# jjhbw/GoMILP

Measured on AMD Instinct MI355X. Metric: simplex pivots/sec on 2048x4096 fp64 dense LP, higher is better.
Workload: dtype f64

## Files before the change

### gomilp_amd/csrc/btg_kernels.hip

```cpp
#include <hip/hip_runtime.h>
#include <hip/hip_ext.h>
#include <stdint.h>

#include <algorithm>
#include <type_traits>

#include "device_types.h"
#include "kernels_common.h"
#include "bt_loop.h"

namespace gomilp {

namespace {

struct XWin { double m; unsigned int i; double p0, p1, p2, p3; };
struct BtWinG { double m; unsigned int i; };

}

template <int G, int NT, int RI, int KR, bool STAMP, bool LOOP = false>
__device__ __forceinline__ void bt_innerG_body(const BTArgs &a, const int g, const int nupd = 0) {
    constexpr int NW = NT / 64;
    static_assert(!LOOP || KR == 16 || KR == 24 || KR == 32, "loop mode: KR / 2 lagging + KR / 2 current terms");
    constexpr int KB = LOOP ? KR / 2 : KR;
    static_assert(G == 2 || G == 4 || G == 8 || G == 16, "G");
#ifdef GOMILP_DEBUG
    if (a.fault && g == 1) return;
#endif
    __shared__ double redM[16];
    __shared__ unsigned int redI[16];
    __shared__ double pay[16][4];
    __shared__ int s_ok;
    __shared__ unsigned long long s_acc[STAMP ? 16 : 1][16];
    unsigned long long tprev = 0;
    auto stamp = [&](int seg) {
        if constexpr (STAMP) {
            unsigned long long t;
            __builtin_amdgcn_sched_barrier(0);
            asm volatile("s_memtime %0\n\ts_waitcnt lgkmcnt(0)" : "=s"(t)::"memory");
            __builtin_amdgcn_sched_barrier(0);
            if (seg >= 0 && (threadIdx.x & 63) == 0) s_acc[threadIdx.x >> 6][seg] += t - tprev;
            tprev = t;
        }
    };
    DevState *st = a.st;
    const int tid = threadIdx.x, lane = tid & 63, wv = tid >> 6;
    const int wbase = __builtin_amdgcn_readfirstlane(tid & ~63);
    const int done = __hip_atomic_load(&st->done, __ATOMIC_RELAXED, __HIP_MEMORY_SCOPE_AGENT);
    long long xs = (long long)a.xbuf[0];
    xpair *recs = reinterpret_cast<xpair *>(a.xbuf + kXHeader);
    const double inf = __builtin_inf();
    const unsigned int ldt = (unsigned int)a.ldt;
    const char *Tb = reinterpret_cast<const char *>(a.T);
    auto ldT = [&](unsigned int elem) -> double {
        if constexpr (LOOP) return ld_agent(reinterpret_cast<const double *>(Tb + (elem << 3)));
        else return *reinterpret_cast<const double *>(Tb + (elem << 3));
    };
    auto ld_term = [&](const double *p) -> double { return ld_agent(p); };
    auto st_term = [&](double *p, double v) { st_agent(p, v); };
    auto gidx = [&](int s) -> int { return (s * G + g) * NT + tid; };
    unsigned int myxcc;
    asm volatile("s_getreg_b32 %0, hwreg(HW_REG_XCC_ID)" : "=s"(myxcc));
    myxcc &= 0xFu;
    bool fast = false, first = true;
    double xbv[RI], rv[RI];
    int basv[RI], nbasv[RI];
#pragma unroll
    for (int s = 0; s < RI; s++) {
        const int i = gidx(s);
        xbv[s] = i < a.m ? a.xb[i] : 0.0;
        basv[s] = i < a.m ? a.basic[i] : 0;
        rv[s] = i < a.nn ? a.r[i] : inf;
        nbasv[s] = i < a.nn ? a.nonbasic[i] : 0;
    }
    int cur0 = 0, lag0 = KB, nl = 0;
    const int sel0 = LOOP ? (a.par ? st->tsel2[1] : st->tsel2[0]) : 0;
    const double *hdr_in = a.xbuf + 1 + 5 * (LOOP ? a.par : 0);
    double *hdr_out = a.xbuf + 1 + 5 * (LOOP ? (a.par ^ 1) : 0);
    const unsigned int blk_base = LOOP ? (unsigned int)(unsigned long long)hdr_in[0] : 0u;
    unsigned int upd_base[4];
#pragma unroll
    for (int j = 0; j < 4; j++) upd_base[j] = LOOP ? (unsigned int)(unsigned long long)hdr_in[1 + j] : 0u;
    unsigned int *blk_cnt = reinterpret_cast<unsigned int *>(a.xbuf + kXSync), *upd_cnt = reinterpret_cast<unsigned int *>(a.xbuf + kXSync + 16);
    auto hand_on = [&](int nb) {
        hdr_out[0] = (double)(unsigned int)(blk_base + (unsigned int)G * (unsigned int)nb);
#pragma unroll
        for (int j = 0; j < 4; j++) hdr_out[1 + j] = (double)(unsigned int)(upd_base[j] + (unsigned int)nupd * (unsigned int)(nb > j ? (nb - 1 - j) / 4 + 1 : 0));
    };
    if (done) {
        if constexpr (LOOP) {
            if (tid == 0) {
                if (g == 0) {
                    __hip_atomic_store(&st->kdone2[0], 0, __ATOMIC_RELAXED, __HIP_MEMORY_SCOPE_AGENT);
                    asm volatile("s_waitcnt vmcnt(0)" ::: "memory");
                }
                __hip_atomic_fetch_add(blk_cnt, 1u, __ATOMIC_RELAXED, __HIP_MEMORY_SCOPE_AGENT);
                if (g == 0) {
                    st->tsel2[a.par ^ 1] = sel0;
                    st->loop_blocks = 0;
                    hand_on(1);
                }
            }
        } else if (g == 0 && tid == 0) st->kdone = 0;
        return;
    }
    double ureg[RI][KR], vreg[RI][KR];
#pragma unroll
    for (int s = 0; s < RI; s++) {
#pragma unroll
        for (int j = 0; j < KR; j++) { ureg[s][j] = 0; vreg[s][j] = 0; }
    }
    if constexpr (STAMP) { if (tid < 256) s_acc[tid >> 4][tid & 15] = 0; }
    __syncthreads();
    int kd = 0, status = ST_RUNNING, blands = 0;
    bool dead = false;
    long long trace_len = 0, npiv = 0;
    if (g == 0 && tid == 0) { trace_len = st->trace_len; npiv = st->pivots; }

    auto wave_first_min = [&](const double (&val)[RI]) -> BtWinG {
        double x = val[0];
#pragma unroll
        for (int s = 1; s < RI; s++) x = vmin_f64(x, val[s]);
        BtWinG w;
        w.m = wave_min_f64(x);
        w.i = 0xFFFFFFFFu;
#pragma unroll
        for (int s = RI - 1; s >= 0; s--) {
            const unsigned long long mask = __ballot(val[s] == w.m);
            if (mask) w.i = (unsigned int)((s * G + g) * NT + wbase + __builtin_ctzll(mask));
        }
        return w;
    };
    auto xchg = [&](int which) -> XWin {
        stamp(which * 5 + 0);
        if constexpr (!LOOP) asm volatile("s_waitcnt vmcnt(0)" ::: "memory");
        __syncthreads();
        stamp(which * 5 + 1);
        xs += 1;
        const double seqd = (double)xs;
        const int par = (int)(xs & 1);
        if (wv == 0) {
            double fm, v0;
            unsigned int fi;
            if constexpr (LOOP && (NW == 4 || NW == 8)) {
                const double mw = lane < NW ? redM[lane & (NW - 1)] : inf;
                const double iw = lane < NW ? (double)redI[lane & (NW - 1)] : 4294967295.0;
                double xm = mw;
                xm = vmin_f64(xm, dpp_f64<0xB1>(xm));
                xm = vmin_f64(xm, dpp_f64<0x4E>(xm));
                if constexpr (NW == 8) xm = vmin_f64(xm, dpp_f64<0x141>(xm));
                const bool mine = lane < NW && mw == xm;
                double km = mine ? iw : 4294967295.0;
                km = vmin_f64(km, dpp_f64<0xB1>(km));
                km = vmin_f64(km, dpp_f64<0x4E>(km));
                if constexpr (NW == 8) km = vmin_f64(km, dpp_f64<0x141>(km));
                const unsigned int mk = (unsigned int)(__ballot(mine && iw == km) & ((1ull << NW) - 1ull));
                const int ww = mk ? __builtin_ctz(mk) : 0;
                fm = readlane_f64(mw, ww);
                fi = (unsigned int)readlane_f64(iw, ww);
                v0 = pay[ww][lane < 5 && lane >= 2 ? lane - 2 : 3];
            } else {
                fm = redM[0];
                fi = redI[0];
                v0 = pay[0][lane < 5 && lane >= 2 ? lane - 2 : 3];
#pragma unroll
                for (int w2 = 1; w2 < NW; w2++) {
                    const double mw = redM[w2];
                    const unsigned int iw = redI[w2];
                    const double pw = pay[w2][lane < 5 && lane >= 2 ? lane - 2 : 3];
                    const bool take = (mw < fm) || (mw == fm && iw < fi) || (fm != fm && mw == mw);
                    fm = take ? mw : fm;
                    fi = take ? iw : fi;
                    v0 = take ? pw : v0;
                }
            }
            if (lane < kXSlots) {
                xpair v;
                v.x = seqd;
                v.y = lane == 0 ? fm : lane == 1 ? (double)fi : lane == 5 ? (double)myxcc : v0;
                xstore(recs + ((size_t)(par * G + g) * kXSlots + lane), v, fast);
            }
            if constexpr (STAMP && !LOOP) asm volatile("s_waitcnt vmcnt(0)" ::: "memory");
        }
        stamp(which * 5 + 2);
        for (int dl = 0; dl < a.poll_delay; dl++) __builtin_amdgcn_s_sleep(1);
        if constexpr (G == 16) {
            const int rec = lane & 15, grp = lane >> 4;
            const bool actB = grp < 3;
            const xpair *base = recs + (size_t)par * G * kXSlots + rec * kXSlots;
            const xpair *srcA = base + (grp == 0 ? 0 : grp + 1), *srcB = base + (grp == 0 ? 1 : grp == 1 ? 5 : grp == 2 ? 6 : 0);
            xpair got[2];
            int spins = 0;
            for (;;) {
                XLoad<2>::run(srcA, srcB, got, fast);
                if (__all(got[0].x == seqd && (!actB || got[1].x == seqd))) break;
                if (++spins > kXSpinLimit) { dead = true; break; }
            }
            stamp(which * 5 + 3);
            const double val = got[0].y, val2 = got[1].y;
            double xm = (lane < 16) ? val : inf;
            xm = vmin_f64(xm, dpp_f64<0xB1>(xm));
            xm = vmin_f64(xm, dpp_f64<0x4E>(xm));
            xm = vmin_f64(xm, dpp_f64<0x141>(xm));
            xm = vmin_f64(xm, dpp_f64<0x140>(xm));
            const bool mine = lane < 16 && val == xm;
            const unsigned int mk0 = (unsigned int)(__ballot(mine) & 0xFFFFull);
            int gw;
            double bi;
            if (__builtin_popcount(mk0) == 1) {
                gw = __builtin_ctz(mk0);
                bi = readlane_f64(val2, gw);
            } else {
                double km = mine ? val2 : 4294967295.0;
                km = vmin_f64(km, dpp_f64<0xB1>(km));
                km = vmin_f64(km, dpp_f64<0x4E>(km));
                km = vmin_f64(km, dpp_f64<0x141>(km));
                km = vmin_f64(km, dpp_f64<0x140>(km));
                const unsigned int mk = (unsigned int)(__ballot(mine && val2 == km) & 0xFFFFull);
                gw = mk ? __builtin_ctz(mk) : 0;
                bi = readlane_f64(km, 0);
            }
            XWin r;
            r.m = readlane_f64(xm, 0);
            r.i = (unsigned int)bi;
            r.p0 = readlane_f64(val, 16 + gw);
            r.p1 = readlane_f64(val, 32 + gw);
            r.p2 = readlane_f64(val, 48 + gw);
            r.p3 = readlane_f64(val2, 32 + gw);
            if (first) {
                fast = !dead && __all(grp != 1 || val2 == (double)myxcc);
                first = false;
            }
            stamp(which * 5 + 4);
            return r;
        }
        const bool act = (lane & 7) < G && (lane >> 3) < 7;
        const xpair *src = recs + (size_t)par * G * kXSlots + (act ? (lane & 7) * kXSlots + (lane >> 3) : 0);
        xpair got[1];
        int spins = 0;
        for (;;) {
            XLoad<1>::run(src, got, fast);
            if (__all(!act || got[0].x == seqd)) break;
            if (++spins > kXSpinLimit) { dead = true; break; }
        }
        stamp(which * 5 + 3);
        const double val = got[0].y;
        double xm = (lane < G) ? val : inf;
        xm = vmin_f64(xm, dpp_f64<0xB1>(xm));
        xm = vmin_f64(xm, dpp_f64<0x4E>(xm));
        xm = vmin_f64(xm, dpp_f64<0x141>(xm));
        const double idxl = dpp_f64<0x108>(val);
        const bool mine = lane < G && val == xm;
        double km = mine ? idxl : 4294967295.0;
        km = vmin_f64(km, dpp_f64<0xB1>(km));
        km = vmin_f64(km, dpp_f64<0x4E>(km));
        km = vmin_f64(km, dpp_f64<0x141>(km));
        const unsigned int mk = (unsigned int)(__ballot(mine && idxl == km) & 0xFFull);
        const int gw = mk ? __builtin_ctz(mk) : 0;
        const double bm = readlane_f64(xm, 0), bi = readlane_f64(km, 0);
        XWin r;
        r.m = bm;
        r.i = (unsigned int)bi;
        r.p0 = readlane_f64(val, 16 + gw);
        r.p1 = readlane_f64(val, 24 + gw);
        r.p2 = readlane_f64(val, 32 + gw);
        r.p3 = readlane_f64(val, 48 + gw);
        if (first) {
            fast = !dead && __all(!(act && (lane >> 3) == 5) || val == (double)myxcc);
            first = false;
        }
        stamp(which * 5 + 4);
        return r;
    };
    auto reduce_cols = [&](const double (&val)[RI]) -> XWin {
        const BtWinG w = wave_first_min(val);
#pragma unroll
        for (int s = 0; s < RI; s++)
            if ((unsigned int)gidx(s) == w.i) {
                pay[wv][0] = rv[s];
                pay[wv][1] = (double)nbasv[s];
                pay[wv][3] = vreg[s][0];
            }
        if (lane == 0) { redM[wv] = w.m; redI[wv] = w.i; }
        return xchg(0);
    };
    auto reduce_rows = [&](const double (&val)[RI], const double (&dcol)[RI]) -> XWin {
        const BtWinG w = wave_first_min(val);
#pragma unroll
        for (int s = 0; s < RI; s++)
            if ((unsigned int)gidx(s) == w.i) {
                pay[wv][0] = dcol[s];
                pay[wv][1] = xbv[s];
                pay[wv][2] = (double)basv[s];
                pay[wv][3] = ureg[s][0];
            }
        if (lane == 0) { redM[wv] = w.m; redI[wv] = w.i; }
        return xchg(1);
    };
    auto column = [&](int q, int k, double (&dcol)[RI], double newest) {
        double d0[RI];
#pragma unroll
        for (int s = 0; s < RI; s++) {
            const int i = gidx(s);
            const unsigned int ic = (unsigned int)(i < a.m ? i : a.m - 1);
            d0[s] = ldT(tile_off_g(ic, (unsigned int)q, ldt));
        }
        double vq[KR];
        if constexpr (LOOP) {
            const int l = lane & 31;
            const int trow = l < k ? cur0 + k - 1 - l : lag0 + nl - 1 - (l - k);
            double tv = l < k + nl ? ld_term(a.V + (size_t)trow * a.ldt + q) : 0.0;
            if (l == 0 && k + nl > 0) tv = newest;
            if constexpr (STAMP) { asm volatile("s_waitcnt vmcnt(0)" ::: "memory"); stamp(11); }
#pragma unroll
            for (int jj = 0; jj < KR; jj++) vq[jj] = readlane_f64(tv, jj);
        } else {
#pragma unroll
            for (int jj = 0; jj < KR; jj++) vq[jj] = jj < k ? ld_term(a.V + (size_t)(k - 1 - jj) * a.ldt + q) : 0.0;
        }
#pragma unroll
        for (int s = 0; s < RI; s++) {
            double d;
            if constexpr (LOOP) {
                double acc[4] = {0, 0, 0, 0};
#pragma unroll
                for (int j = 0; j < KR; j++) acc[j & 3] = __builtin_fma(ureg[s][j], vq[j], acc[j & 3]);
                d = d0[s] + ((acc[0] + acc[1]) + (acc[2] + acc[3]));
            } else {
                d = d0[s];
#pragma unroll
                for (int j = 0; j < KR; j++) d = __builtin_fma(ureg[s][j], vq[j], d);
            }
            dcol[s] = gidx(s) < a.m ? d : 0.0;
        }
    };
    auto ratios = [&](const double (&dcol)[RI], double (&mvv)[RI]) {
#pragma unroll
        for (int s = 0; s < RI; s++) {
            const int i = gidx(s);
            double d = -dcol[s];
            if (fabs(d) < 1e-13) d = 0;
            const double quot = div_pos(xbv[s], fabs(d));
            mvv[s] = (d >= 0 || i >= a.m) ? inf : quot;
        }
    };

    int nbe = 0;
    for (int blk = 0; blk < (LOOP ? a.nblocks : 1); blk++) {
    if constexpr (LOOP) {
        if (blk >= 2) {
            if (wv == 0) {
                const int cj = (blk - 2) & 3;
                const unsigned int ub = cj == 0 ? upd_base[0] : cj == 1 ? upd_base[1] : cj == 2 ? upd_base[2] : upd_base[3];
                const bool ok = spin_counter(upd_cnt + 16 * cj * 2, ub + (unsigned int)nupd * (unsigned int)((blk - 2) / 4 + 1), 0);
                if (lane == 0) s_ok = ok ? 1 : 0;
            }
            __syncthreads();
            if (!s_ok) { dead = true; break; }
        }
        Tb = reinterpret_cast<const char *>(((sel0 ^ (blk > 0 ? blk - 1 : 0)) & 1) ? a.Tbuf[1] : a.Tbuf[0]);
        cur0 = (blk & 1) * KB; lag0 = cur0 ^ KB; nl = blk > 0 ? KB : 0;
        if (blk > 0) {
#pragma unroll
            for (int s = 0; s < RI; s++) {
#pragma unroll
                for (int j = KB; j < KR; j++) { ureg[s][j] = 0; vreg[s][j] = 0; }
            }
        }
        kd = 0;
    }
    for (int k = 0; k < a.kmax; k++) {
        stamp(-1);
        const bool forced = (k == 0 && blk == 0 && a.forced_q >= 0);
        int q, p, ent = 0, lea = 0;
        double rq = 0, dpv = 1.0, xbp = 0, unew = 0;
        bool bland = false;
        double dcol[RI];
        if (!forced) {
            const XWin fq = reduce_cols(rv);
            if (dead) break;
            q = (int)fq.i; rq = fq.p0; ent = (int)fq.p1;
            if (fq.i >= (unsigned int)a.nn) { q = 0; rq = __builtin_nan(""); }
            if (a.guard == inf && !(k == 0 && blk == 0 && a.exact_once)) { status = ST_NEED_EXACT; break; }
            if (rq >= -a.tol) { status = ST_OPTIMAL; break; }
            column(q, k, dcol, fq.p3);
            XWin w;
            {
                double mvv[RI];
                ratios(dcol, mvv);
                w = reduce_rows(mvv, dcol);
            }
            if (dead) break;
            p = (int)w.i; dpv = w.p0; xbp = w.p1; lea = (int)w.p2; unew = w.p3;
            const double mv = w.m;
            if (mv == inf || w.i >= (unsigned int)a.m) { status = ST_UNBOUNDED; break; }
            if (a.guard > 0 && (mv <= a.guard || fabs(dpv) <= a.guard) && !(k == 0 && blk == 0 && a.exact_once)) { status = ST_NEED_EXACT; break; }
            if (a.cguard > 0 && fabs(dpv) <= a.cguard && !(k == 0 && blk == 0 && a.exact_once)) { status = ST_NEED_EXACT; break; }
            if (mv <= 0) {
                bland = true;
                blands++;
                int cand = -1;
                bool found = false;
                for (;;) {
                    double fl[RI];
#pragma unroll
                    for (int s = 0; s < RI; s++) {
                        const int j = gidx(s);
                        double rr = rv[s];
                        if (fabs(rr) < 1e-13) rr = 0;
                        fl[s] = (j < a.nn && j > cand && !(rr > -1e-14)) ? 0.0 : inf;
                    }
                    const XWin fc = reduce_cols(fl);
                    if (dead) break;
                    if (fc.m != 0.0) break;
                    cand = (int)fc.i;
                    const double rqc = fc.p0;
                    const int entc = (int)fc.p1;
                    column(cand, k, dcol, fc.p3);
                    XWin w2;
                    {
                        double mvv[RI];
                        ratios(dcol, mvv);
                        w2 = reduce_rows(mvv, dcol);
                    }
                    if (dead) break;
                    if (w2.m == inf || w2.i >= (unsigned int)a.m) { status = ST_UNBOUNDED; break; }
                    if (fabs(w2.m) > 1e-12) {
                        q = cand; p = (int)w2.i; rq = rqc; ent = entc; dpv = w2.p0; xbp = w2.p1; lea = (int)w2.p2; unew = w2.p3;
                        found = true;
                        break;
                    }
                    double gl2[RI];
                    ratios(dcol, gl2);
#pragma unroll
                    for (int s = 0; s < RI; s++) gl2[s] = (gidx(s) < a.m && !(gl2[s] > 1e-12)) ? 0.0 : inf;
                    const XWin gw = reduce_rows(gl2, dcol);
                    if (dead) break;
                    if (gw.m == 0.0) {
                        q = cand; p = (int)gw.i; rq = rqc; ent = entc; dpv = gw.p0; xbp = gw.p1; lea = (int)gw.p2; unew = gw.p3;
                        found = true;
                        break;
                    }
                }
                if (dead || status == ST_UNBOUNDED) break;
                if (!found) { status = ST_BLAND_FAILED; break; }
            }
        } else {
            q = a.forced_q; p = a.forced_p; rq = 0;
            double fl[RI];
#pragma unroll
            for (int s = 0; s < RI; s++) fl[s] = (gidx(s) == q) ? 0.0 : inf;
            const XWin fc = reduce_cols(fl);
            if (dead) break;
            ent = (int)fc.p1;
            if (!a.forced_nocommit) rq = fc.p0;
            column(q, k, dcol, fc.p3);
            double gl2[RI];
#pragma unroll
            for (int s = 0; s < RI; s++) gl2[s] = (gidx(s) == p) ? 0.0 : inf;
            const XWin gw = reduce_rows(gl2, dcol);
            if (dead) break;
            dpv = gw.p0; xbp = gw.p1; lea = (int)gw.p2; unew = gw.p3;
        }
        const double rinv = 1.0 / dpv, nrinv = -rinv;
        const double mult = rq * rinv;
        const double theta = xbp * rinv;
        double *Vk = a.V + (size_t)(cur0 + k) * a.ldt;
        double *Uk = a.U + (size_t)(cur0 + k) * a.ldu;
        const bool commit_lists = !(forced && a.forced_nocommit) || (forced && a.forced_nocommit >= 2);
        double vrow[RI];
#pragma unroll
        for (int s = 0; s < RI; s++) {
            const int j = gidx(s);
            vrow[s] = j < a.ldt ? ldT(tile_off_g((unsigned int)p, (unsigned int)j, ldt)) : 0.0;
        }
        double up[KR];
        if constexpr (LOOP) {
            const int l = lane & 31;
            const int trow = l < k ? cur0 + k - 1 - l : lag0 + nl - 1 - (l - k);
            double tv = l < k + nl ? ld_term(a.U + (size_t)trow * a.ldu + p) : 0.0;
            if (l == 0 && k + nl > 0) tv = unew;
            if constexpr (STAMP) { asm volatile("s_waitcnt vmcnt(0)" ::: "memory"); stamp(12); }
#pragma unroll
            for (int jj = 0; jj < KR; jj++) up[jj] = readlane_f64(tv, jj);
        } else {
#pragma unroll
            for (int jj = 0; jj < KR; jj++) up[jj] = jj < k ? ld_term(a.U + (size_t)(k - 1 - jj) * a.ldu + p) : 0.0;
        }
        if constexpr (LOOP) asm volatile("s_waitcnt vmcnt(0)" ::: "memory");
#pragma unroll
        for (int s = 0; s < RI; s++) {
            const int i = gidx(s);
            if (i < a.ldu) {
                const double u = (i == p) ? rinv - 1.0 : dcol[s] * nrinv;
                if (i < a.m) xbv[s] = (i == p) ? theta : __builtin_fma(-theta, dcol[s], xbv[s]);
                st_term(Uk + i, u);
#pragma unroll
                for (int jj = KR - 1; jj > 0; jj--) ureg[s][jj] = ureg[s][jj - 1];
                ureg[s][0] = u;
                if (i == p && commit_lists) basv[s] = ent;
            }
        }
#pragma unroll
        for (int s = 0; s < RI; s++) {
            const int j = gidx(s);
            if (j < a.ldt) {
                double v;
                if constexpr (LOOP) {
                    double acc[4] = {0, 0, 0, 0};
#pragma unroll
                    for (int jj = 0; jj < KR; jj++) acc[jj & 3] = __builtin_fma(up[jj], vreg[s][jj], acc[jj & 3]);
                    v = vrow[s] + ((acc[0] + acc[1]) + (acc[2] + acc[3]));
                } else {
                    v = vrow[s];
#pragma unroll
                    for (int jj = 0; jj < KR; jj++) v = __builtin_fma(up[jj], vreg[s][jj], v);
                }
                rv[s] = (j == q) ? -mult : __builtin_fma(-mult, v, rv[s]);
                const double vprime = (j == q) ? dpv + 1.0 : v;
                st_term(Vk + j, vprime);
#pragma unroll
                for (int jj = KR - 1; jj > 0; jj--) vreg[s][jj] = vreg[s][jj - 1];
                vreg[s][0] = vprime;
                if (j == q && commit_lists) nbasv[s] = lea;
            }
        }
        if constexpr (STAMP && !LOOP) asm volatile("s_waitcnt vmcnt(0)" ::: "memory");
        stamp(10);
        if (forced && a.forced_nocommit == 3) status = ST_FORCED_DONE;
        if (g == 0 && tid == 0 && !(forced && a.forced_nocommit)) {
            if (a.trace && trace_len < a.trace_cap) {
                DevPivot &tr = a.trace[trace_len];
                tr.phase = a.phase; tr.bland = bland ? 1 : 0; tr.min_idx = q; tr.replace = p; tr.entering = ent; tr.leaving = lea;
            }
            trace_len += 1;
            npiv += 1;
        }
        kd = k + 1;
    }
    nbe = blk + 1;
    if constexpr (LOOP) {
        if (dead) status = ST_XCHG_TIMEOUT;
        asm volatile("s_waitcnt vmcnt(0)" ::: "memory");
        __syncthreads();
        if (tid == 0) {
            if (g == 0) {
                __hip_atomic_store(&st->kdone2[blk & 1], kd, __ATOMIC_RELAXED, __HIP_MEMORY_SCOPE_AGENT);
                if (status != ST_RUNNING) {
                    __hip_atomic_store(&st->status, status, __ATOMIC_RELAXED, __HIP_MEMORY_SCOPE_AGENT);
                    __hip_atomic_store(&st->done, 1, __ATOMIC_RELAXED, __HIP_MEMORY_SCOPE_AGENT);
                }
                asm volatile("s_waitcnt vmcnt(0)" ::: "memory");
            }
            __hip_atomic_fetch_add(blk_cnt, 1u, __ATOMIC_RELAXED, __HIP_MEMORY_SCOPE_AGENT);
        }
        if (status != ST_RUNNING) break;
    }
    }
    if (dead) status = ST_XCHG_TIMEOUT;
    if constexpr (STAMP) {
        if (a.stamps && g == 0 && lane == 0) {
            for (int sg = 0; sg < 16; sg++) a.stamps[wv * 16 + sg] += s_acc[wv][sg];
            if (wv == 0) a.stamps[16 * 16] += (unsigned long long)kd;
        }
    }
#pragma unroll
    for (int s = 0; s < RI; s++) {
        const int i = gidx(s);
        if (i < a.ldt) a.r[i] = i < a.nn ? rv[s] : 0.0;
        if (i < a.ldu) a.xb[i] = xbv[s];
        if (i < a.m) a.basic[i] = basv[s];
        if (i < a.nn) a.nonbasic[i] = nbasv[s];
    }
    if (tid == 0 && (g == 0 || dead)) {
        if (g == 0) {
            st->trace_len = trace_len;
            st->pivots = npiv;
            if constexpr (LOOP) {
                const int napplied = kd > 0 ? nbe : nbe - 1;
                st->tsel2[a.par ^ 1] = sel0 ^ (napplied & 1);
                st->loop_blocks = nbe;
                hand_on(nbe);
            } else {
                st->kdone = kd;
            }
            st->bland_steps += blands;
            a.xbuf[0] = (double)xs;
        }
        if (status != ST_RUNNING) { st->done = 1; st->status = status; }
    }
}

template <int G, int NT, int RI, int KR, bool STAMP = false>
__global__ __launch_bounds__(NT) void k_bt_innerG(BTArgs a) {
    if (blockIdx.x & 7u) return;
    bt_innerG_body<G, NT, RI, KR, STAMP>(a, (int)(blockIdx.x >> 3));
}
template <int G, int NT, int RI, bool STAMP = false, int KB = 8>
__global__ __launch_bounds__(NT) void k_bt_loop(BTArgs a) {
    const int b = (int)blockIdx.x, x = a.xcd & 7;
    const int nupd = (a.upd_cap > 0 && a.upd_cap < (int)gridDim.x - G) ? a.upd_cap : (int)gridDim.x - G;
    if ((b & 7) == x && (b >> 3) < G) { bt_innerG_body<G, NT, RI, 2 * KB, STAMP, true>(a, b >> 3, nupd); return; }
    const int before = b <= x ? 0 : min(G, ((b - x - 1) >> 3) + 1);
    if (b - before >= nupd) return;
    bt_loop_update_role<NT, KB>(a, b - before, nupd, G);
}

template <int G, int NT, int RI, int KR>
__global__ __launch_bounds__(NT) void k_bt_innerG_batch(const BatchLP *__restrict__ lps, const int *__restrict__ ids, const int *__restrict__ count, int xcd_off) {
    const unsigned int x8 = ((blockIdx.x & 7u) + 8u - (unsigned int)xcd_off) & 7u, j = blockIdx.x >> 3;
    const int lpos = (int)((j / G) * 8u + x8);
    if (lpos >= *count) return;
    const BatchLP &lp = lps[ids[lpos]];
    const int stage = lp.stage;
    if (stage == BS_DONE || stage == BS_HOST) return;
    const BTArgs a = lp.bt;
    bt_innerG_body<G, NT, RI, KR, false>(a, (int)(j % G));
}


size_t bt_xbuf_doubles() { return (size_t)kXSync + kXSyncDoubles; }

BtGroupCfg bt_group_cfg(int m, int ldt, int knob) {
    BtGroupCfg c = {0, 0, 0};
    if (knob < 0) return c;
    const int need = m > ldt ? m : ldt;
    auto fits = [&](int G, int nt, int ri) { return (long)G * nt * ri >= need; };
    if (knob == 16) {
        if (need <= 2048) c = {8, 256, 1};
        else if (need <= 4096) c = {8, 512, 1};
        return c;
    }
    if (knob == 2 || knob == 4 || knob == 8) {
        const int G = knob;
        if (fits(G, 512, 1)) c = {G, 512, 1};
        else if (fits(G, 512, 2)) c = {G, 512, 2};
        return c;
    }
    if (knob != 0) return c;
    if (need <= 1024) return c;
    if (need <= 2048) return {8, 256, 1};
    if (need <= 4096) return {8, 512, 1};
    if (need <= 8192) return {8, 512, 2};
    return c;
}

template <int G, int NT, int RI>
static void btg_launch(const BTArgs &a, hipStream_t s, hipEvent_t e0, hipEvent_t e1) {
    if constexpr (RI == 1) {
        if (a.stamps) { hipExtLaunchKernelGGL((k_bt_innerG<G, NT, RI, 16, true>), dim3(8 * G), dim3(NT), 0, s, e0, e1, 0, a); return; }
    }
    hipExtLaunchKernelGGL((k_bt_innerG<G, NT, RI, 16>), dim3(8 * G), dim3(NT), 0, s, e0, e1, 0, a);
}
void launch_bt_inner_groups(const BTArgs &a, hipStream_t s, hipEvent_t e0, hipEvent_t e1) {
    const int G = a.groups, ri = a.group_ri;
// ... 35 lines not shown
```

### gomilp_amd/csrc/kernels_common.h

```cpp
#pragma once
#include <hip/hip_runtime.h>
#include <stdint.h>

#include "device_types.h"

#include <mutex>
#include <set>
#include <utility>

namespace gomilp {

inline void lds_attr_once(const void *fn, int bytes) {
    static std::mutex mu;
    static std::set<std::pair<int, const void *>> done;
    int dev = 0;
    (void)hipGetDevice(&dev);
    std::lock_guard<std::mutex> g(mu);
    if (done.insert(std::make_pair(dev, fn)).second) (void)hipFuncSetAttribute(fn, hipFuncAttributeMaxDynamicSharedMemorySize, bytes);
}

static inline int grid_for_rows(int rows) {
    int g = (rows + kWavesPerBlock - 1) / kWavesPerBlock;
    if (g > kMaxPartials) g = kMaxPartials;
    if (g < 1) g = 1;
// ... 105 lines not shown
    if (b.k < a.k || (b.k == a.k && b.i < a.i)) a = b;
}
__device__ __forceinline__ void wave_argminp(ArgMinP &a) {
#pragma unroll
    for (int o = 32; o > 0; o >>= 1) {
        ArgMinP b;
        b.k = __shfl_xor(a.k, o, 64); b.i = __shfl_xor(a.i, o, 64); b.u = __shfl_xor(a.u, o, 64); b.d = __shfl_xor(a.d, o, 64);
        aminp_take(a, b);
    }
}
__device__ __forceinline__ void block_argminp(ArgMinP &a, ArgMinP *sm) {
    wave_argminp(a);
    const int w = threadIdx.x >> 6;
    if ((threadIdx.x & 63) == 0) sm[w] = a;
    __syncthreads();
    a = sm[0];
#pragma unroll
    for (int t = 1; t < kWavesPerBlock; t++) aminp_take(a, sm[t]);
    __syncthreads();
}

struct BtCand {
    unsigned long long k;
    unsigned int i;
};
__device__ __forceinline__ void bt_take(BtCand &a, const BtCand &b) {
    if (b.k < a.k || (b.k == a.k && b.i < a.i)) a = b;
}
template <int CTRL>
__device__ __forceinline__ unsigned int dpp_u32(unsigned int v) {
    return (unsigned int)__builtin_amdgcn_update_dpp((int)v, (int)v, CTRL, 0xF, 0xF, false);
}
template <int CTRL>
__device__ __forceinline__ BtCand dpp_cand(const BtCand &a) {
    BtCand b;
    const unsigned int klo = dpp_u32<CTRL>((unsigned int)a.k), khi = dpp_u32<CTRL>((unsigned int)(a.k >> 32));
    b.k = ((unsigned long long)khi << 32) | klo;
    b.i = dpp_u32<CTRL>(a.i);
    return b;
}
__device__ __forceinline__ BtCand readlane_cand(const BtCand &a, int lane) {
    BtCand b;
    const unsigned int klo = (unsigned int)__builtin_amdgcn_readlane((int)(unsigned int)a.k, lane);
    const unsigned int khi = (unsigned int)__builtin_amdgcn_readlane((int)(unsigned int)(a.k >> 32), lane);
    b.k = ((unsigned long long)khi << 32) | klo;
    b.i = (unsigned int)__builtin_amdgcn_readlane((int)a.i, lane);
    return b;
}
__device__ __forceinline__ void row_argmin(BtCand &a) {
    bt_take(a, dpp_cand<0x111>(a));
    bt_take(a, dpp_cand<0x112>(a));
    bt_take(a, dpp_cand<0x114>(a));
    bt_take(a, dpp_cand<0x118>(a));
}
template <int NW>
__device__ __forceinline__ void bt_block_argmin(BtCand &a, BtCand *sm) {
    row_argmin(a);
    BtCand w = readlane_cand(a, 15);
    bt_take(w, readlane_cand(a, 31));
    bt_take(w, readlane_cand(a, 47));
    bt_take(w, readlane_cand(a, 63));
    const int wv = threadIdx.x >> 6, lane = threadIdx.x & 63;
    if (lane == 0) sm[wv] = w;
    __syncthreads();
    BtCand c;
    c.k = ~0ull; c.i = 0xFFFFFFFFu;
    if (lane < NW) c = sm[lane];
    row_argmin(c);
    a = readlane_cand(c, 15);
}

template <int CTRL>
__device__ __forceinline__ double dpp_f64(double v) {
    const unsigned long long b = (unsigned long long)__double_as_longlong(v);
    const unsigned int lo = dpp_u32<CTRL>((unsigned int)b), hi = dpp_u32<CTRL>((unsigned int)(b >> 32));
    return __longlong_as_double((long long)(((unsigned long long)hi << 32) | lo));
}
__device__ __forceinline__ double readlane_f64(double v, int lane) {
    const unsigned long long b = (unsigned long long)__double_as_longlong(v);
    const unsigned int lo = (unsigned int)__builtin_amdgcn_readlane((int)(unsigned int)b, lane);
    const unsigned int hi = (unsigned int)__builtin_amdgcn_readlane((int)(unsigned int)(b >> 32), lane);
    return __longlong_as_double((long long)(((unsigned long long)hi << 32) | lo));
}
__device__ __forceinline__ double vmin_f64(double a, double b) {
    double r;
    asm("v_min_f64 %0, %1, %2" : "=v"(r) : "v"(a), "v"(b));
    return r;
}
template <int CTRL>
__device__ __forceinline__ unsigned int ror_u32(unsigned int v) {
    return (unsigned int)__builtin_amdgcn_mov_dpp((int)v, CTRL, 0xF, 0xF, false);
}
template <int CTRL>
__device__ __forceinline__ double ror_f64(double v) {
    const unsigned long long b = (unsigned long long)__double_as_longlong(v);
    const unsigned int lo = ror_u32<CTRL>((unsigned int)b), hi = ror_u32<CTRL>((unsigned int)(b >> 32));
    return __longlong_as_double((long long)(((unsigned long long)hi << 32) | lo));
}
__device__ __forceinline__ double row_min_f64(double x) {
    x = vmin_f64(x, ror_f64<0x121>(x));
    x = vmin_f64(x, ror_f64<0x122>(x));
    x = vmin_f64(x, ror_f64<0x124>(x));
    x = vmin_f64(x, ror_f64<0x128>(x));
    return x;
}
template <int CTRL, int ROWMASK>
__device__ __forceinline__ double bcast_f64(double v) {
    const unsigned long long b = (unsigned long long)__double_as_longlong(v);
    const unsigned int lo = (unsigned int)__builtin_amdgcn_update_dpp((int)(unsigned int)b, (int)(unsigned int)b, CTRL, ROWMASK, 0xF, false);
    const unsigned int hi = (unsigned int)__builtin_amdgcn_update_dpp((int)(unsigned int)(b >> 32), (int)(unsigned int)(b >> 32), CTRL, ROWMASK, 0xF, false);
    return __longlong_as_double((long long)(((unsigned long long)hi << 32) | lo));
}
__device__ __forceinline__ double wave_min_f64(double x) {
    x = row_min_f64(x);
    x = vmin_f64(x, bcast_f64<0x142, 0xA>(x));
    x = vmin_f64(x, bcast_f64<0x143, 0xC>(x));
    return readlane_f64(x, 63);
}
__device__ __forceinline__ unsigned int row_min_u32(unsigned int x) {
    x = min(x, ror_u32<0x121>(x));
    x = min(x, ror_u32<0x122>(x));
    x = min(x, ror_u32<0x124>(x));
    x = min(x, ror_u32<0x128>(x));
    return x;
}

__device__ __forceinline__ double div_pos(double x, double d) {
    double r = __builtin_amdgcn_rcp(d);
    double e = __builtin_fma(-d, r, 1.0);
    r = __builtin_fma(r, e, r);
    e = __builtin_fma(-d, r, 1.0);
    r = __builtin_fma(r, e, r);
    double q = x * r;
    const double rem = __builtin_fma(-d, q, x);
    return __builtin_fma(rem, r, q);
}

__device__ __forceinline__ size_t tab_idx(int i, int j, int ldt, int tiled) {
    return tiled ? ((size_t)(i >> 2) * (size_t)(ldt >> 2) + (size_t)(j >> 2)) * 16u + (size_t)(((i & 3) << 2) + (j & 3))
                 : (size_t)i * ldt + j;
}

__device__ __forceinline__ void stage_vec(double2 *__restrict__ svec, const double *__restrict__ src, int ld2) {
    const double2 *s2 = reinterpret_cast<const double2 *>(src);
    for (int c = threadIdx.x; c < ld2; c += kBlock) svec[c] = s2[c];
    __syncthreads();
}

struct DotAcc {
    double a0, a1, a2, a3;
};

template <int NV>
__device__ __forceinline__ void wave_dot_chunk(const double *__restrict__ row, const double2 *__restrict__ svec, int sstride, int c0,
                                               int c1, int ld2, int lane, DotAcc (&acc)[NV]) {
    const double2 *r2 = reinterpret_cast<const double2 *>(row);
    int c = c0 + lane;
    for (; c + 192 < c1; c += 256) {
        const double2 v0 = r2[c], v1 = r2[c + 64], v2 = r2[c + 128], v3 = r2[c + 192];
#pragma unroll
        for (int v = 0; v < NV; v++) {
            const double2 *s = svec + v * sstride + (c - c0);
            const double2 s0 = s[0], s1 = s[64], s2 = s[128], s3 = s[192];
            acc[v].a0 += v0.x * s0.x + v0.y * s0.y;
            acc[v].a1 += v1.x * s1.x + v1.y * s1.y;
            acc[v].a2 += v2.x * s2.x + v2.y * s2.y;
// ... 80 lines not shown
```

Measured before the change: 211,100.

## Broadcast eta terms via DPP row_bcast and pin kernel args to SGPRs

In loop mode, the lagging and current eta terms are no longer broadcast with per-term readlane into scalar registers. Each 16-lane row now loads them and broadcasts them through DPP row_newbcast into VGPRs, disabled for the NT=512/KR=32 configuration. Kernel arguments (m, nn, ldt, V, U, tol and so on) are forced through v_mov plus readfirstlane copies so they stay in SGPRs rather than being reloaded from the kernarg segment. The U/V update loops are split and reordered with unsigned row-offset arithmetic. The aim is to cut SALU/readlane serialisation and scalar reloads on the per-pivot critical path, at the cost of more VGPR pressure and extra vector loads of the terms.

```diff
diff --git a/gomilp_amd/csrc/btg_kernels.hip b/gomilp_amd/csrc/btg_kernels.hip
--- a/gomilp_amd/csrc/btg_kernels.hip
+++ b/gomilp_amd/csrc/btg_kernels.hip
@@ -23,6 +23,7 @@
     constexpr int NW = NT / 64;
     static_assert(!LOOP || KR == 16 || KR == 24 || KR == 32, "loop mode: KR / 2 lagging + KR / 2 current terms");
     constexpr int KB = LOOP ? KR / 2 : KR;
+    constexpr bool ROWB = LOOP && !(NT == 512 && KR == 32);
     static_assert(G == 2 || G == 4 || G == 8 || G == 16, "G");
 #ifdef GOMILP_DEBUG
     if (a.fault && g == 1) return;
@@ -43,6 +44,39 @@
             tprev = t;
         }
     };
+    auto own32 = [](unsigned int x) -> unsigned int {
+        unsigned int t;
+        asm volatile("v_mov_b32 %0, %1" : "=v"(t) : "s"(x));
+        return (unsigned int)__builtin_amdgcn_readfirstlane((int)t);
+    };
+    auto own = [&](const auto &v) -> decltype(auto) {
+        if constexpr (LOOP) {
+            typedef std::remove_cv_t<std::remove_reference_t<decltype(v)>> T;
+            if constexpr (sizeof(T) == 8) {
+                const unsigned long long b = __builtin_bit_cast(unsigned long long, v);
+                const unsigned long long r = ((unsigned long long)own32((unsigned int)(b >> 32)) << 32) | own32((unsigned int)b);
+                return __builtin_bit_cast(T, r);
+            } else {
+                return __builtin_bit_cast(T, own32(__builtin_bit_cast(unsigned int, v)));
+            }
+        } else {
+            return (v);
+        }
+    };
+    auto own_ptr = [&](auto *const &ptr) -> decltype(auto) {
+        if constexpr (LOOP) {
+            typedef std::remove_pointer_t<std::remove_cv_t<std::remove_reference_t<decltype(ptr)>>> T;
+            typedef __attribute__((address_space(1))) T GT;
+            return (T *)(GT *)own((unsigned long long)ptr);
+        } else {
+            return (ptr);
+        }
+    };
+    std::conditional_t<LOOP, const int, const int &> a_m = own(a.m), a_nn = own(a.nn), a_ldt = own(a.ldt), a_ldu = own(a.ldu), a_kmax = own(a.kmax), a_poll_delay = own(a.poll_delay);
+    std::conditional_t<LOOP, double *const, double *const &> a_V = own_ptr(a.V), a_U = own_ptr(a.U);
+    std::conditional_t<LOOP, const double, const double &> a_tol = own(a.tol), a_guard = own(a.guard), a_cguard = own(a.cguard);
+    std::conditional_t<LOOP, DevPivot *const, DevPivot *const &> a_trace = own_ptr(a.trace);
+    std::conditional_t<LOOP, const int64_t, const int64_t &> a_trace_cap = own(a.trace_cap);
     DevState *st = a.st;
     const int tid = threadIdx.x, lane = tid & 63, wv = tid >> 6;
     const int wbase = __builtin_amdgcn_readfirstlane(tid & ~63);
@@ -50,7 +84,7 @@
     long long xs = (long long)a.xbuf[0];
     xpair *recs = reinterpret_cast<xpair *>(a.xbuf + kXHeader);
     const double inf = __builtin_inf();
-    const unsigned int ldt = (unsigned int)a.ldt;
+    const unsigned int ldt = (unsigned int)a_ldt;
     const char *Tb = reinterpret_cast<const char *>(a.T);
     auto ldT = [&](unsigned int elem) -> double {
         if constexpr (LOOP) return ld_agent(reinterpret_cast<const double *>(Tb + (elem << 3)));
@@ -68,10 +102,10 @@
 #pragma unroll
     for (int s = 0; s < RI; s++) {
         const int i = gidx(s);
-        xbv[s] = i < a.m ? a.xb[i] : 0.0;
-        basv[s] = i < a.m ? a.basic[i] : 0;
-        rv[s] = i < a.nn ? a.r[i] : inf;
-        nbasv[s] = i < a.nn ? a.nonbasic[i] : 0;
+        xbv[s] = i < a_m ? a.xb[i] : 0.0;
+        basv[s] = i < a_m ? a.basic[i] : 0;
+        rv[s] = i < a_nn ? a.r[i] : inf;
+        nbasv[s] = i < a_nn ? a.nonbasic[i] : 0;
     }
     int cur0 = 0, lag0 = KB, nl = 0;
     const int sel0 = LOOP ? (a.par ? st->tsel2[1] : st->tsel2[0]) : 0;
@@ -183,7 +217,7 @@
             if constexpr (STAMP && !LOOP) asm volatile("s_waitcnt vmcnt(0)" ::: "memory");
         }
         stamp(which * 5 + 2);
-        for (int dl = 0; dl < a.poll_delay; dl++) __builtin_amdgcn_s_sleep(1);
+        for (int dl = 0; dl < a_poll_delay; dl++) __builtin_amdgcn_s_sleep(1);
         if constexpr (G == 16) {
             const int rec = lane & 15, grp = lane >> 4;
             const bool actB = grp < 3;
@@ -302,21 +336,33 @@
 #pragma unroll
         for (int s = 0; s < RI; s++) {
             const int i = gidx(s);
-            const unsigned int ic = (unsigned int)(i < a.m ? i : a.m - 1);
+            const unsigned int ic = (unsigned int)(i < a_m ? i : a_m - 1);
             d0[s] = ldT(tile_off_g(ic, (unsigned int)q, ldt));
         }
         double vq[KR];
         if constexpr (LOOP) {
-            const int l = lane & 31;
-            const int trow = l < k ? cur0 + k - 1 - l : lag0 + nl - 1 - (l - k);
-            double tv = l < k + nl ? ld_term(a.V + (size_t)trow * a.ldt + q) : 0.0;
-            if (l == 0 && k + nl > 0) tv = newest;
-            if constexpr (STAMP) { asm volatile("s_waitcnt vmcnt(0)" ::: "memory"); stamp(11); }
-#pragma unroll
-            for (int jj = 0; jj < KR; jj++) vq[jj] = readlane_f64(tv, jj);
+            if constexpr (ROWB) {
+                double tv[2] = {0.0, 0.0};
+#pragma unroll
+                for (int h = 0; h < (KR > 16 ? 2 : 1); h++) {
+                    const int l = (lane & 15) + 16 * h;
+                    const int trow = l < k ? cur0 + k - 1 - l : lag0 + nl - 1 - (l - k);
+                    tv[h] = l < k + nl ? ld_term(a_V + (size_t)trow * a_ldt + q) : 0.0;
+                }
+                if ((lane & 15) == 0 && k + nl > 0) tv[0] = newest;
+                if constexpr (STAMP) { asm volatile("s_waitcnt vmcnt(0)" ::: "memory"); stamp(11); }
+                row_bcast_terms<KR>(vq, tv[0], tv[1]);
+            } else {
+                const int l = lane & 31;
+                const int trow = l < k ? cur0 + k - 1 - l : lag0 + nl - 1 - (l - k);
+                double tv = l < k + nl ? ld_term(a_V + (size_t)trow * a_ldt + q) : 0.0;
+                if (l == 0 && k + nl > 0) tv = newest;
+#pragma unroll
+                for (int jj = 0; jj < KR; jj++) vq[jj] = readlane_f64(tv, jj);
+            }
         } else {
 #pragma unroll
-            for (int jj = 0; jj < KR; jj++) vq[jj] = jj < k ? ld_term(a.V + (size_t)(k - 1 - jj) * a.ldt + q) : 0.0;
+            for (int jj = 0; jj < KR; jj++) vq[jj] = jj < k ? ld_term(a_V + (size_t)(k - 1 - jj) * a_ldt + q) : 0.0;
         }
 #pragma unroll
         for (int s = 0; s < RI; s++) {
@@ -331,7 +377,7 @@
 #pragma unroll
                 for (int j = 0; j < KR; j++) d = __builtin_fma(ureg[s][j], vq[j], d);
             }
-            dcol[s] = gidx(s) < a.m ? d : 0.0;
+            dcol[s] = gidx(s) < a_m ? d : 0.0;
         }
     };
     auto ratios = [&](const double (&dcol)[RI], double (&mvv)[RI]) {
@@ -341,7 +387,7 @@
             double d = -dcol[s];
             if (fabs(d) < 1e-13) d = 0;
             const double quot = div_pos(xbv[s], fabs(d));
-            mvv[s] = (d >= 0 || i >= a.m) ? inf : quot;
+            mvv[s] = (d >= 0 || i >= a_m) ? inf : quot;
         }
     };
 
@@ -369,7 +415,7 @@
         }
         kd = 0;
     }
-    for (int k = 0; k < a.kmax; k++) {
+    for (int k = 0; k < a_kmax; k++) {
         stamp(-1);
         const bool forced = (k == 0 && blk == 0 && a.forced_q >= 0);
         int q, p, ent = 0, lea = 0;
@@ -380,9 +426,9 @@
             const XWin fq = reduce_cols(rv);
             if (dead) break;
             q = (int)fq.i; rq = fq.p0; ent = (int)fq.p1;
-            if (fq.i >= (unsigned int)a.nn) { q = 0; rq = __builtin_nan(""); }
-            if (a.guard == inf && !(k == 0 && blk == 0 && a.exact_once)) { status = ST_NEED_EXACT; break; }
-            if (rq >= -a.tol) { status = ST_OPTIMAL; break; }
+            if (fq.i >= (unsigned int)a_nn) { q = 0; rq = __builtin_nan(""); }
+            if (a_guard == inf && !(k == 0 && blk == 0 && a.exact_once)) { status = ST_NEED_EXACT; break; }
+            if (rq >= -a_tol) { status = ST_OPTIMAL; break; }
             column(q, k, dcol, fq.p3);
             XWin w;
             {
@@ -393,9 +439,9 @@
             if (dead) break;
             p = (int)w.i; dpv = w.p0; xbp = w.p1; lea = (int)w.p2; unew = w.p3;
             const double mv = w.m;
-            if (mv == inf || w.i >= (unsigned int)a.m) { status = ST_UNBOUNDED; break; }
-            if (a.guard > 0 && (mv <= a.guard || fabs(dpv) <= a.guard) && !(k == 0 && blk == 0 && a.exact_once)) { status = ST_NEED_EXACT; break; }
-            if (a.cguard > 0 && fabs(dpv) <= a.cguard && !(k == 0 && blk == 0 && a.exact_once)) { status = ST_NEED_EXACT; break; }
+            if (mv == inf || w.i >= (unsigned int)a_m) { status = ST_UNBOUNDED; break; }
+            if (a_guard > 0 && (mv <= a_guard || fabs(dpv) <= a_guard) && !(k == 0 && blk == 0 && a.exact_once)) { status = ST_NEED_EXACT; break; }
+            if (a_cguard > 0 && fabs(dpv) <= a_cguard && !(k == 0 && blk == 0 && a.exact_once)) { status = ST_NEED_EXACT; break; }
             if (mv <= 0) {
                 bland = true;
                 blands++;
@@ -408,7 +454,7 @@
                         const int j = gidx(s);
                         double rr = rv[s];
                         if (fabs(rr) < 1e-13) rr = 0;
-                        fl[s] = (j < a.nn && j > cand && !(rr > -1e-14)) ? 0.0 : inf;
+                        fl[s] = (j < a_nn && j > cand && !(rr > -1e-14)) ? 0.0 : inf;
                     }
                     const XWin fc = reduce_cols(fl);
                     if (dead) break;
@@ -424,7 +470,7 @@
                         w2 = reduce_rows(mvv, dcol);
                     }
                     if (dead) break;
-                    if (w2.m == inf || w2.i >= (unsigned int)a.m) { status = ST_UNBOUNDED; break; }
+                    if (w2.m == inf || w2.i >= (unsigned int)a_m) { status = ST_UNBOUNDED; break; }
                     if (fabs(w2.m) > 1e-12) {
                         q = cand; p = (int)w2.i; rq = rqc; ent = entc; dpv = w2.p0; xbp = w2.p1; lea = (int)w2.p2; unew = w2.p3;
                         found = true;
@@ -433,7 +479,7 @@
                     double gl2[RI];
                     ratios(dcol, gl2);
 #pragma unroll
-                    for (int s = 0; s < RI; s++) gl2[s] = (gidx(s) < a.m && !(gl2[s] > 1e-12)) ? 0.0 : inf;
+                    for (int s = 0; s < RI; s++) gl2[s] = (gidx(s) < a_m && !(gl2[s] > 1e-12)) ? 0.0 : inf;
                     const XWin gw = reduce_rows(gl2, dcol);
                     if (dead) break;
                     if (gw.m == 0.0) {
@@ -465,72 +511,107 @@
         const double rinv = 1.0 / dpv, nrinv = -rinv;
         const double mult = rq * rinv;
         const double theta = xbp * rinv;
-        double *Vk = a.V + (size_t)(cur0 + k) * a.ldt;
-        double *Uk = a.U + (size_t)(cur0 + k) * a.ldu;
+        double *Vk = a_V + (LOOP ? (size_t)((unsigned int)(cur0 + k) * (unsigned int)a_ldt) : (size_t)(cur0 + k) * a_ldt);
+        double *Uk = a_U + (LOOP ? (size_t)((unsigned int)(cur0 + k) * (unsigned int)a_ldu) : (size_t)(cur0 + k) * a_ldu);
         const bool commit_lists = !(forced && a.forced_nocommit) || (forced && a.forced_nocommit >= 2);
         double vrow[RI];
 #pragma unroll
         for (int s = 0; s < RI; s++) {
             const int j = gidx(s);
-            vrow[s] = j < a.ldt ? ldT(tile_off_g((unsigned int)p, (unsigned int)j, ldt)) : 0.0;
+            vrow[s] = j < a_ldt ? ldT(tile_off_g((unsigned int)p, (unsigned int)j, ldt)) : 0.0;
         }
         double up[KR];
         if constexpr (LOOP) {
-            const int l = lane & 31;
-            const int trow = l < k ? cur0 + k - 1 - l : lag0 + nl - 1 - (l - k);
-            double tv = l < k + nl ? ld_term(a.U + (size_t)trow * a.ldu + p) : 0.0;
-            if (l == 0 && k + nl > 0) tv = unew;
-            if constexpr (STAMP) { asm volatile("s_waitcnt vmcnt(0)" ::: "memory"); stamp(12); }
-#pragma unroll
-            for (int jj = 0; jj < KR; jj++) up[jj] = readlane_f64(tv, jj);
+            if constexpr (ROWB) {
+                double tv[2] = {0.0, 0.0};
+#pragma unroll
+                for (int h = 0; h < (KR > 16 ? 2 : 1); h++) {
+                    const int l = (lane & 15) + 16 * h;
+                    const int trow = l < k ? cur0 + k - 1 - l : lag0 + nl - 1 - (l - k);
+                    tv[h] = l < k + nl ? ld_term(a_U + (size_t)trow * a_ldu + p) : 0.0;
+                }
+                if ((lane & 15) == 0 && k + nl > 0) tv[0] = unew;
+                if constexpr (STAMP) { asm volatile("s_waitcnt vmcnt(0)" ::: "memory"); stamp(12); }
+                row_bcast_terms<KR>(up, tv[0], tv[1]);
+            } else {
+                const int l = lane & 31;
+                const int trow = l < k ? cur0 + k - 1 - l : lag0 + nl - 1 - (l - k);
+                double tv = l < k + nl ? ld_term(a_U + (size_t)trow * a_ldu + p) : 0.0;
+                if (l == 0 && k + nl > 0) tv = unew;
+#pragma unroll
+                for (int jj = 0; jj < KR; jj++) up[jj] = readlane_f64(tv, jj);
+            }
         } else {
 #pragma unroll
-            for (int jj = 0; jj < KR; jj++) up[jj] = jj < k ? ld_term(a.U + (size_t)(k - 1 - jj) * a.ldu + p) : 0.0;
+            for (int jj = 0; jj < KR; jj++) up[jj] = jj < k ? ld_term(a_U + (size_t)(k - 1 - jj) * a_ldu + p) : 0.0;
         }
         if constexpr (LOOP) asm volatile("s_waitcnt vmcnt(0)" ::: "memory");
-#pragma unroll
-        for (int s = 0; s < RI; s++) {
-            const int i = gidx(s);
-            if (i < a.ldu) {
+        if constexpr (LOOP) {
+#pragma unroll
+            for (int s = 0; s < RI; s++) {
+                int j = gidx(s);
+                asm volatile("" : "+v"(j));
+                double acc[4] = {0, 0, 0, 0};
+#pragma unroll
+                for (int jj = 0; jj < KR; jj++) acc[jj & 3] = __builtin_fma(up[jj], vreg[s][jj], acc[jj & 3]);
+                const double v = vrow[s] + ((acc[0] + acc[1]) + (acc[2] + acc[3]));
+                rv[s] = (j == q) ? -mult : __builtin_fma(-mult, v, rv[s]);
+                const double vprime = (j == q) ? dpv + 1.0 : v;
+                if (j < a_ldt) st_term(Vk + j, vprime);
+#pragma unroll
+                for (int jj = KR - 1; jj > 0; jj--) vreg[s][jj] = vreg[s][jj - 1];
+                vreg[s][0] = vprime;
+                if (j == q && commit_lists) nbasv[s] = lea;
+            }
+#pragma unroll
+            for (int s = 0; s < RI; s++) {
+                int i = gidx(s);
+                asm volatile("" : "+v"(i));
                 const double u = (i == p) ? rinv - 1.0 : dcol[s] * nrinv;
-                if (i < a.m) xbv[s] = (i == p) ? theta : __builtin_fma(-theta, dcol[s], xbv[s]);
-                st_term(Uk + i, u);
+                if (i < a_m) xbv[s] = (i == p) ? theta : __builtin_fma(-theta, dcol[s], xbv[s]);
+                if (i < a_ldu) st_term(Uk + i, u);
 #pragma unroll
                 for (int jj = KR - 1; jj > 0; jj--) ureg[s][jj] = ureg[s][jj - 1];
                 ureg[s][0] = u;
                 if (i == p && commit_lists) basv[s] = ent;
             }
-        }
-#pragma unroll
-        for (int s = 0; s < RI; s++) {
-            const int j = gidx(s);
-            if (j < a.ldt) {
-                double v;
-                if constexpr (LOOP) {
-                    double acc[4] = {0, 0, 0, 0};
-#pragma unroll
-                    for (int jj = 0; jj < KR; jj++) acc[jj & 3] = __builtin_fma(up[jj], vreg[s][jj], acc[jj & 3]);
-                    v = vrow[s] + ((acc[0] + acc[1]) + (acc[2] + acc[3]));
-                } else {
-                    v = vrow[s];
+        } else {
+#pragma unroll
+            for (int s = 0; s < RI; s++) {
+                const int i = gidx(s);
+                if (i < a_ldu) {
+                    const double u = (i == p) ? rinv - 1.0 : dcol[s] * nrinv;
+                    if (i < a_m) xbv[s] = (i == p) ? theta : __builtin_fma(-theta, dcol[s], xbv[s]);
+                    st_term(Uk + i, u);
+#pragma unroll
+                    for (int jj = KR - 1; jj > 0; jj--) ureg[s][jj] = ureg[s][jj - 1];
+                    ureg[s][0] = u;
+                    if (i == p && commit_lists) basv[s] = ent;
+                }
+            }
+#pragma unroll
+            for (int s = 0; s < RI; s++) {
+                const int j = gidx(s);
+                if (j < a_ldt) {
+                    double v = vrow[s];
 #pragma unroll
                     for (int jj = 0; jj < KR; jj++) v = __builtin_fma(up[jj], vreg[s][jj], v);
-                }
-                rv[s] = (j == q) ? -mult : __builtin_fma(-mult, v, rv[s]);
-                const double vprime = (j == q) ? dpv + 1.0 : v;
-                st_term(Vk + j, vprime);
-#pragma unroll
-                for (int jj = KR - 1; jj > 0; jj--) vreg[s][jj] = vreg[s][jj - 1];
-                vreg[s][0] = vprime;
-                if (j == q && commit_lists) nbasv[s] = lea;
+                    rv[s] = (j == q) ? -mult : __builtin_fma(-mult, v, rv[s]);
+                    const double vprime = (j == q) ? dpv + 1.0 : v;
+                    st_term(Vk + j, vprime);
+#pragma unroll
+                    for (int jj = KR - 1; jj > 0; jj--) vreg[s][jj] = vreg[s][jj - 1];
+                    vreg[s][0] = vprime;
+                    if (j == q && commit_lists) nbasv[s] = lea;
+                }
             }
         }
         if constexpr (STAMP && !LOOP) asm volatile("s_waitcnt vmcnt(0)" ::: "memory");
         stamp(10);
         if (forced && a.forced_nocommit == 3) status = ST_FORCED_DONE;
         if (g == 0 && tid == 0 && !(forced && a.forced_nocommit)) {
-            if (a.trace && trace_len < a.trace_cap) {
-                DevPivot &tr = a.trace[trace_len];
+            if (a_trace && trace_len < a_trace_cap) {
+                DevPivot &tr = a_trace[trace_len];
                 tr.phase = a.phase; tr.bland = bland ? 1 : 0; tr.min_idx = q; tr.replace = p; tr.entering = ent; tr.leaving = lea;
             }
             trace_len += 1;
@@ -567,10 +648,10 @@
 #pragma unroll
     for (int s = 0; s < RI; s++) {
         const int i = gidx(s);
-        if (i < a.ldt) a.r[i] = i < a.nn ? rv[s] : 0.0;
-        if (i < a.ldu) a.xb[i] = xbv[s];
-        if (i < a.m) a.basic[i] = basv[s];
-        if (i < a.nn) a.nonbasic[i] = nbasv[s];
+        if (i < a_ldt) a.r[i] = i < a_nn ? rv[s] : 0.0;
+        if (i < a_ldu) a.xb[i] = xbv[s];
+        if (i < a_m) a.basic[i] = basv[s];
+        if (i < a_nn) a.nonbasic[i] = nbasv[s];
     }
     if (tid == 0 && (g == 0 || dead)) {
         if (g == 0) {
diff --git a/gomilp_amd/csrc/kernels_common.h b/gomilp_amd/csrc/kernels_common.h
--- a/gomilp_amd/csrc/kernels_common.h
+++ b/gomilp_amd/csrc/kernels_common.h
@@ -211,6 +211,18 @@
     const unsigned int hi = (unsigned int)__builtin_amdgcn_readlane((int)(unsigned int)(b >> 32), lane);
     return __longlong_as_double((long long)(((unsigned long long)hi << 32) | lo));
 }
+template <int N>
+__device__ __forceinline__ double row_bcast_f64(double v) {
+    static_assert(N >= 0 && N < 16, "lane of the row");
+    return __builtin_amdgcn_update_dpp(0.0, v, 0x150 + N, 0xF, 0xF, true);
+}
+template <int KR, int J = 0>
+__device__ __forceinline__ void row_bcast_terms(double (&out)[KR], double lo, double hi) {
+    if constexpr (J < KR) {
+        out[J] = row_bcast_f64<(J & 15)>(J < 16 ? lo : hi);
+        row_bcast_terms<KR, J + 1>(out, lo, hi);
+    }
+}
 __device__ __forceinline__ double vmin_f64(double a, double b) {
     double r;
     asm("v_min_f64 %0, %1, %2" : "=v"(r) : "v"(a), "v"(b));
```

New measurement: 219,300 (median of 6 runs). 3.9% higher.
